# k-flouris/cmf

Hardware: AMD Instinct MI355X
Metric: log-density evals/sec (JtJ-cholesky path), MNIST D=784 d=64 bs=512 (higher is better)
Workload: dtype f32 (3x3 tangent convs as bf16x3 split MFMA, fp32 accumulate); 1 GPU; C3: MNIST-shaped (1,28,28) uint8-range + U[0,1) noise, non-square flow d=64, cholesky J^T J log-det + g_ij off-diagonal L1 + reconstruction, eval/no_grad; per_gpu_batch=512, global_batch=512, D=784, latent_dimension=64, parallelism=dp1

## Files before the change

### cmf_amd/_lib.py

```python
import ctypes as C
import os
import threading

_HERE = os.path.dirname(os.path.abspath(__file__))
LIB_PATH = os.path.join(_HERE, "libcmf_amd.so")

F_NONE, F_RELU, F_TANH, F_RAW, F_SELF_RELU, F_RELU_BITS = 0, 1, 2, 3, 4, 5
O_NONE, O_TANH, O_STANH = 0, 1, 2
GRAM_INVALID, GRAM_RING64, GRAM_DIRECT128, GRAM_WIDE, GRAM_RING_LIMIT = 0, 64, 128, 512, 0x7fffff00

_fp = C.c_void_p
_ll = C.c_longlong
_i = C.c_int
_f = C.c_float
_d = C.c_double


class ConvTangentArgs(C.Structure):
    _fields_ = [("x", _fp), ("x_np", _ll), ("x_ci", _ll), ("x_px", _ll),
                ("f", _fp), ("f_np", _ll), ("f_ci", _ll), ("f_px", _ll), ("fmode", _i),
                ("w", _fp),
                ("y", _fp), ("y_np", _ll), ("y_co", _ll), ("y_px", _ll),
                ("r", _fp), ("r_np", _ll), ("r_co", _ll), ("r_px", _ll),
                ("np", _i), ("cin", _i), ("cout", _i), ("H", _i), ("W", _i), ("nc", _i), ("taps", _i),
                ("bias", _fp), ("f_group", _i), ("x_sl", _ll), ("y_sl", _ll), ("r_sl", _ll),
                ("fo", _fp), ("fo_np", _ll), ("fo_co", _ll), ("fo_px", _ll), ("fomode", _i),
                ("mask_out", _fp), ("mask_np", _ll), ("amax_in", _fp), ("amax_out", _fp), ("live", _i),
                ("ymask", _fp), ("ymask_np", _ll),
                ("head_w", _fp), ("head_cout", _i), ("head_a", _fp), ("head_a_np", _ll), ("head_a_c", _ll), ("head_a_px", _ll),
                ("head_y", _fp), ("head_y_np", _ll), ("head_y_co", _ll), ("head_y_px", _ll),
                ("seed", _fp), ("seed_np", _ll), ("seed_col", _ll), ("seed_w", _fp),
                ("block_w1", _fp), ("block_m1", _fp), ("block_m1_np", _ll)]


class ConvPrimalArgs(C.Structure):
    _fields_ = [("x", _fp), ("x_b", _ll), ("x_c", _ll), ("x_px", _ll),
                ("f", _fp), ("f_c", _ll), ("f_px", _ll), ("imode", _i),
                ("w", _fp), ("bias", _fp), ("sw", _fp), ("sb", _fp),
                ("y", _fp), ("y_b", _ll), ("y_c", _ll), ("y_px", _ll),
                ("g", _fp),
                ("r", _fp), ("r_b", _ll), ("r_c", _ll), ("r_px", _ll),
                ("omode", _i),
                ("B", _i), ("cin", _i), ("cout", _i), ("H", _i), ("W", _i), ("taps", _i)]


class ProbeApplyArgs(C.Structure):
    _fields_ = [("r", _fp), ("r_np", _ll), ("r_px", _ll),
                ("t", _fp), ("t_np", _ll), ("t_c", _ll), ("t_px", _ll),
                ("cls", _fp),
                ("y", _fp), ("y_np", _ll), ("y_px", _ll),
                ("ymask", _fp), ("ymask_np", _ll),
                ("np", _i), ("cin", _i), ("H", _i), ("W", _i), ("nc", _i), ("ns", _i)]


MLP_MAX_LAYERS = 8
WGRAD_MAX_BATCH = 16


class MlpCouplerArgs(C.Structure):
    _fields_ = [("z", _fp), ("z_b", _ll), ("t", _fp), ("t_f", _ll), ("w", _fp),
                ("zi", _fp), ("si", _fp), ("ti", _fp), ("n_mod", _i),
                ("B", _i), ("cin", _i), ("chan_off", _i), ("chan_step", _i), ("n_layers", _i),
                ("width", _i * (MLP_MAX_LAYERS + 1)), ("w_off", _ll * MLP_MAX_LAYERS), ("decode", _i), ("lj", _fp), ("ncols", _i)]


SIGNATURES = {
    "cmf_version": (C.c_char_p, []),
    "cmf_pack_weight": (_i, [_fp, _fp, _i, _i, _i, _i, C.POINTER(_ll), _fp]),
    "cmf_pack_weights_batched": (_i, [_fp, _i, _fp]),
    "cmf_conv_tangent": (_i, [C.POINTER(ConvTangentArgs), _fp]),
    "cmf_pack_weight_bf16x3": (_i, [_fp, _fp, _i, _i, C.POINTER(_ll), _fp]),
    "cmf_pack_weight_bf16x3_t": (_i, [_fp, _fp, _i, _i, _i, C.POINTER(_ll), _fp]),
    "cmf_conv_tangent_bf16x3": (_i, [C.POINTER(ConvTangentArgs), _fp]),
    "cmf_probe_apply": (_i, [C.POINTER(ProbeApplyArgs), _fp]),
    "cmf_pack_seed_weight": (_i, [_fp, _fp, _fp]),
    "cmf_seed_panel": (_i, [_fp, _ll, _ll, _fp, _fp, _ll, _ll, _i, _i, _i, _i, _fp]),
    "cmf_pack_block_weight": (_i, [_fp, _fp, C.POINTER(_ll), _fp]),
    "cmf_pack_weight_f16x3": (_i, [_fp, _fp, _i, _i, _i, C.POINTER(_ll), _fp]),
    "cmf_conv_tangent_f16x3": (_i, [C.POINTER(ConvTangentArgs), _fp]),
    "cmf_conv_tangent_f16x3_item": (_i, [C.POINTER(ConvTangentArgs), _i, _fp]),
    "cmf_absmax": (_i, [_fp, _ll, _fp, _fp]),
    "cmf_conv_tangent_wgrad_ws": (_ll, [C.POINTER(ConvTangentArgs)]),
    "cmf_conv_tangent_wgrad": (_i, [C.POINTER(ConvTangentArgs), _fp, _fp, _fp, _ll, _fp]),
    "cmf_conv_tangent_wgrad_bf16x3": (_i, [C.POINTER(ConvTangentArgs), _fp, _fp, _fp, _ll, _fp]),
    "cmf_conv_tangent_wgrad_bf16x3_batched": (_i, [C.POINTER(ConvTangentArgs), _i, C.POINTER(_fp), C.POINTER(_fp), C.POINTER(_fp), _fp, _ll, _fp]),
    "cmf_primal_regroup": (_i, [_fp, _fp, _i, _ll, _i, _fp]),
    "cmf_conv_primal": (_i, [C.POINTER(ConvPrimalArgs), _fp]),
    "cmf_acl_primal": (_i, [_fp, _ll, _fp, _ll, _fp, _fp, _fp, _i, _i, _i, _fp, _fp]),
    "cmf_acl_tangent": (_i, [_fp, _ll, _ll, _fp, _ll, _ll, _i, _fp, _ll, _fp, _ll, _fp, _fp, _fp, _fp, _i, _i, _fp]),
    "cmf_acl_cotangent": (_i, [_fp, _ll, _ll, _fp, _ll, _ll, _i, _fp, _ll, _fp, _ll, _fp, _fp, _fp, _fp, _i, _i, _fp]),
    "cmf_acl_primal_backward": (_i, [_fp, _ll, _fp, _ll, _fp, _ll, _fp, _fp, _fp, _fp, _i, _i, _i, _fp, _fp]),
    "cmf_acl_cross_terms": (_i, [_fp, _ll, _ll, _fp, _ll, _ll, _fp, _ll, _ll, _i, _fp, _ll, _fp, _ll, _fp, _fp, _fp, _fp, _i, _i,
                            _fp, _fp, _fp, _fp]),
    "cmf_gather_primal": (_i, [_fp, _ll, _fp, _ll, _fp, _i, _i, _fp]),
    "cmf_gather_tangent": (_i, [_fp, _ll, _ll, _fp, _ll, _ll, _fp, _i, _i, _i, _fp]),
    "cmf_seed_tangent": (_i, [_fp, _ll, _ll, _fp, _i, _i, _fp, _i, _i, _i, _fp]),
    "cmf_gram_cholesky": (_i, [_fp, _ll, _ll, _i, _i, _i, _i, _fp, _fp, _fp, _fp, _fp, _fp, _fp]),
    "cmf_cholesky_retry": (_i, [_fp, _i, _i, _i, _f, _fp, _fp, _fp, _fp, _fp]),
    "cmf_gram_cholesky_family": (_i, [_i, _i, _ll]),
    "cmf_gram_condition": (_i, [_fp, _fp, _i, _i, _f, _fp, _fp, _fp, _fp, _fp]),
    "cmf_metric_stats_ws": (_ll, [_i, _i, _i, _i]),
    "cmf_metric_stats_accumulate": (_i, [_fp, _i, _i, _i, _fp, _fp, _ll, _fp, _fp]),
    "cmf_gram_spectrum": (_i, [_fp, _i, _i, _fp, _fp, _fp, _fp, _fp]),
    "cmf_gauss_newton_step": (_i, [_fp, _ll, _ll, _i, _i, _i, _i, _fp, _fp, _fp, _fp, _fp, _fp, _fp, _fp, _fp]),
    "cmf_cross_gram": (_i, [_fp, _ll, _ll, _i, _i, _i, _i, _i, _fp, _fp]),
    "cmf_curve_step_ws": (_ll, [_i, _i, _i]),
    "cmf_curve_step": (_i, [_fp, _ll, _ll, _i, _i, _i, _i, _i, _fp, _fp, _fp, _fp, _fp, _fp, _fp, _fp, _fp, _fp, _ll, _fp]),
    "cmf_stanh_backward": (_i, [_fp, _fp, _fp, _fp, _fp, _fp, _fp, _fp, _fp, _i, _i, _i, _fp]),
    "cmf_tanh_cross_terms": (_i, [_fp, _ll, _ll, _fp, _ll, _ll, _fp, _fp, _i, _i, _i, _fp]),
    "cmf_tanh_backward": (_i, [_fp, _fp, _fp, _ll, _fp, _fp]),
    "cmf_affine_prior_backward": (_i, [_fp, _ll, _fp, _ll, _fp, _i, _i, _fp, _fp, _fp, _fp]),
    "cmf_accumulate": (_i, [_fp, _fp, _ll, _fp]),
    "cmf_relu_bits": (_i, [_fp, _fp, _i, _i, _i, _fp]),
    "cmf_channel_sum": (_i, [_fp, _ll, _ll, _ll, _ll, _i, _i, _i, _i, _fp, _fp]),
    "cmf_channel_sum_batched": (_i, [C.POINTER(_fp), C.POINTER(_fp), _i, _ll, _ll, _ll, _ll, _i, _i, _i, _i, _fp]),
    "cmf_grad_sqnorm": (_i, [_fp, _ll, _fp, _fp, _fp]),
    "cmf_optimizer_step": (_i, [_i, _fp, _fp, _fp, _fp, _ll, _d, _d, _d, _d, _d, _i, _fp, _f, _fp]),
    "cmf_gram_backward_matrix": (_i, [_fp, _ll, _ll, _i, _i, _i, _i, _fp, _fp, _ll, _ll, _fp]),
    "cmf_gram_backward": (_i, [_fp, _ll, _ll, _i, _i, _i, _i, _fp, _fp, _fp, _fp, _fp, _ll, _ll, _fp]),
    "cmf_gram_backward_ws": (_i, [_fp, _ll, _ll, _i, _i, _i, _i, _fp, _fp, _fp, _fp, _fp, _ll, _ll, _fp, _fp]),
    "cmf_prehead": (_i, [_fp, _fp, _fp, _fp, _f, _f, _i, _i, _i, _fp]),
    "cmf_prehead_inverse": (_i, [_fp, _fp, _f, _f, _i, _ll, _fp]),
    "cmf_expand_columns": (_i, [_fp, _i, _fp, _i, _fp, _ll, _fp]),
    "cmf_gaussian_logprob": (_i, [_fp, _ll, _i, _i, _fp, _fp]),
    "cmf_affine_prior": (_i, [_fp, _ll, _fp, _fp, _i, _i, _i, _fp, _fp]),
    "cmf_recon_sqerr": (_i, [_fp, _fp, _i, _i, _fp, _fp]),
    "cmf_elbo_combine": (_i, [_fp, _fp, _fp, _fp, _fp, _f, _f, _f, _i, _fp, _fp]),
    "cmf_hutch_cg": (_i, [_fp, _fp, _i, _i, _i, _i, _i, _f, _fp, _fp, _fp, _fp, _fp]),
    "cmf_mlp_coupler": (_i, [C.POINTER(MlpCouplerArgs), _fp]),
    "cmf_pack_mlp_layer": (_i, [_fp, _fp, _i, _i, _i, _i, _i, _fp, C.POINTER(_ll), _fp]),
    "cmf_mlp_hidden_tiles": (_i, [_i]),
    "cmf_rq_spline": (_i, [_fp, _ll, _fp, _i, _i, _i, _f, _i, _i, _fp, _ll, _fp, _fp]),
    "cmf_rq_spline_backward": (_i, [_fp, _ll, _fp, _i, _i, _i, _f, _i, _fp, _ll, _fp, _fp, _ll, _fp, _fp]),
    "cmf_lu_backward": (_i, [_fp, _fp, _fp, _fp, _i, _f, _fp, _i, _fp, _fp, _fp, _fp, _fp]),
    "cmf_gaussian_backward": (_i, [_fp, _fp, _i, _i, _fp, _fp]),
    "cmf_lu_weights": (_i, [_fp, _fp, _fp, _i, _f, _fp, _fp, _fp]),
    "cmf_made_mask_weight": (_i, [_fp, _fp, _i, _i, _i, _i, _i, _fp]),
    "cmf_hutch_metric": (_i, [_fp, _i, _i, _i, _fp, _fp, _fp]),
    "cmf_hutch_cotangent": (_i, [_fp, _fp, _fp, _i, _i, _i, _fp, _fp, _fp, _fp, _fp]),
    "cmf_hutch_lowrank_cotangent": (_i, [_fp, _i, _i, _i, _fp, _fp, _i, _fp, _fp]),
}

_lib = None
_tls = threading.local()


class _Traced:

    def __init__(self, lib, sink):
        self._lib, self._sink = lib, sink

    def __getattr__(self, name):
        fn = getattr(self._lib, name)
        if not name.startswith("cmf_"):
            return fn
        import torch

        def call(*args):
            e0, e1 = torch.cuda.Event(enable_timing=True), torch.cuda.Event(enable_timing=True)
            e0.record()
            rc = fn(*args)
            e1.record()
            role = getattr(_tls, "role", None)
            self._sink.append((name + ":" + role if role else name, getattr(_tls, "phase", None), e0, e1))
            return rc
        return call


class trace:

    def __enter__(self):
        self.prev = getattr(_tls, "sink", None)
        _tls.sink = []
        return _tls.sink

    def __exit__(self, *exc):
        _tls.sink = self.prev
        return False


class phase:
    def __init__(self, label):
        self.label = label

    def __enter__(self):
        self.prev = getattr(_tls, "phase", None)
        if self.prev is None:
            _tls.phase = self.label

    def __exit__(self, *exc):
        _tls.phase = self.prev
        return False


def tracing():
    return getattr(_tls, "sink", None) is not None


class role:

    def __init__(self, label):
        self.label = label

    def __enter__(self):
        self.prev = getattr(_tls, "role", None)
        _tls.role = self.label

    def __exit__(self, *exc):
        _tls.role = self.prev
        return False


def load():
    global _lib
    sink = getattr(_tls, "sink", None)
    if _lib is not None:
        return _lib if sink is None else _Traced(_lib, sink)
    if not os.path.exists(LIB_PATH):
        raise RuntimeError(
            f"{LIB_PATH} is missing: the HIP kernels are the only implementation of this path "
            "(no CPU fallback). Build them with `python -m cmf_amd.build`.")
    lib = C.CDLL(LIB_PATH)
    for name, (res, args) in SIGNATURES.items():
        fn = getattr(lib, name)
        fn.restype, fn.argtypes = res, args
    _lib = lib
    return lib
# ... 7 lines not shown
```

### cmf_amd/csrc/probe_front.hip

```cpp
#include <stdint.h>

#include "common.h"

namespace {

constexpr int HID = 64, NT = 256, SLICE = HID * 16;
constexpr int MAXT = 50;
constexpr int MAXCLS = 32;
constexpr int PASS = 64;

__global__ __launch_bounds__(NT) void probe_apply_kernel(cmf_probe_apply_args a, int nitems) {
  __shared__ __attribute__((aligned(16))) float Rs[MAXCLS * HID];
  __shared__ __attribute__((aligned(16))) float Ts[MAXT * PASS];
  __shared__ int tcls[MAXT], toff[MAXT];
  __shared__ int nterm;

  const int per = (nitems + 7) >> 3;
  const int item = (int)(blockIdx.x & 7) * per + (int)(blockIdx.x >> 3);
  if (item >= nitems) return;
  const int H = a.H, W = a.W, HW = H * W;
  const int b = item / HW, p = item - b * HW;
  const int tid = threadIdx.x, lane = tid & 63, wv = tid >> 6;
  const int ncls = a.ns * 16;
  const f32x4 zero = {0.f, 0.f, 0.f, 0.f};

  unsigned long long live = ~0ull;
  if (a.ymask)
    live = *reinterpret_cast<const unsigned long long*>(reinterpret_cast<const unsigned char*>(a.ymask) + (long long)b * a.ymask_np +
                                                        (long long)p * (HID / 8));

  if (wv == 0) {
    int cls = -1, off = 0;
    if (lane < 25 * a.cin) {
      const int w = lane / a.cin, c = lane - w * a.cin;
      const int r = p / W + w / 5 - 2, col = p % W + w % 5 - 2;
      if (r >= 0 && r < H && col >= 0 && col < W) {
        const int q = r * W + col, k = a.cls[c * HW + q];
        if (k >= 0 && k < ncls) {
          cls = k;
          off = (int)(c * a.t_c + q * a.t_px);
        }
      }
    }
    const unsigned long long bal = __ballot(cls >= 0);
    if (cls >= 0) {
      const int pos = __popcll(bal & ((1ull << lane) - 1ull));
      tcls[pos] = cls;
      toff[pos] = off;
    }
    if (lane == 0) nterm = __popcll(bal);
  }

  {
    const int co = tid >> 2, k4 = (tid & 3) * 4;
    const float* rb = a.r + (long long)b * a.r_np + (long long)p * a.r_px + tid * 4;
    for (int s = 0; s < a.ns; ++s) {
      f32x4 v = zero;
      if ((live >> co) & 1) v = *reinterpret_cast<const f32x4*>(rb + s * SLICE);
#pragma unroll
      for (int m = 0; m < 4; ++m) Rs[(s * 16 + k4 + m) * HID + (co & 15) * 4 + (co >> 4)] = v[m];
    }
  }
  __syncthreads();

  const int n = nterm, nsl = a.nc >> 4, cg = lane >> 2, quad = lane & 3;
  const float* tb = a.t + (long long)b * a.t_np;
  for (int s0 = 0; s0 < nsl; s0 += PASS / 16) {
    const int w4 = (nsl - s0 < PASS / 16 ? nsl - s0 : PASS / 16) * 4;
    if (s0) __syncthreads();
    for (int i = tid; i < n * w4; i += NT) {
      const int j = i / w4, x = i - j * w4;
      *reinterpret_cast<f32x4*>(&Ts[j * PASS + 4 * x]) = *reinterpret_cast<const f32x4*>(tb + toff[j] + s0 * 16 + 4 * x);
    }
    __syncthreads();
    const int sl = s0 + wv;
    if (sl >= nsl) continue;
    f32x4 acc[4] = {zero, zero, zero, zero};
    for (int j = 0; j < n; ++j) {
      const f32x4 c4 = *reinterpret_cast<const f32x4*>(&Rs[tcls[j] * HID + cg * 4]);
      const f32x4 t4 = *reinterpret_cast<const f32x4*>(&Ts[j * PASS + wv * 16 + quad * 4]);
#pragma unroll
      for (int i = 0; i < 4; ++i)
#pragma unroll
        for (int k = 0; k < 4; ++k) acc[i][k] = fmaf(c4[i], t4[k], acc[i][k]);
    }
    float* yb = a.y + (long long)b * a.y_np + (long long)p * a.y_px + sl * SLICE + quad * 4;
#pragma unroll
    for (int i = 0; i < 4; ++i) {
      const int co = cg + 16 * i;
      if ((live >> co) & 1) *reinterpret_cast<f32x4*>(yb + co * 16) = acc[i];
    }
  }
}

bool fits_i32(long long v) { return v >= 0 && v <= 0x7fffffffLL; }

}

extern "C" int cmf_probe_apply(const cmf_probe_apply_args* ap, void* stream) {
  if (!ap) return CMF_EINVAL;
  const cmf_probe_apply_args& a = *ap;
  if (!a.r || !a.t || !a.cls || !a.y) return CMF_EINVAL;
  if (a.np <= 0 || a.H <= 0 || a.W <= 0 || a.nc <= 0 || a.nc % 16) return CMF_EINVAL;
  if (a.cin < 1 || 25 * a.cin > MAXT || a.ns < 1 || a.ns * 16 > MAXCLS) return CMF_EINVAL;
  if ((a.r_np | a.r_px | a.t_np | a.t_c | a.t_px | a.y_np | a.y_px) % 4) return CMF_EINVAL;
  if ((uintptr_t)a.r % 16 || (uintptr_t)a.t % 16 || (uintptr_t)a.y % 16) return CMF_EINVAL;
  if (a.r_np < 0 || a.t_np < 0 || a.y_np < 0 || a.t_c < 0) return CMF_EINVAL;
  if (a.r_px < (long long)a.ns * SLICE || a.y_px < (long long)HID * a.nc || a.t_px < a.nc) return CMF_EINVAL;
  const long long HW = (long long)a.H * a.W;
  if (a.ymask && ((uintptr_t)a.ymask % 8 || a.ymask_np % 8 || a.ymask_np < HW * (HID / 8))) return CMF_EINVAL;
  if (HW > (1 << 24) || !fits_i32(a.cin * a.t_c + HW * a.t_px + a.nc)) return CMF_ERANGE;
  const long long nitems = HW * a.np;
  if (nitems > 0x7ffffff0LL) return CMF_ERANGE;
  const int grid = 8 * (int)((nitems + 7) / 8);
  hipLaunchKernelGGL(probe_apply_kernel, dim3(grid), dim3(NT), 0, (hipStream_t)stream, a, (int)nitems);
  CMF_LAUNCH_CHECK();
  return 0;
}
```

### cmf_amd/engine.py

```python
import ctypes as C
import threading
from typing import NamedTuple

import numpy as np
import torch
import torch.nn as nn

from . import _lib
from ._lib import (F_NONE, F_RELU, F_TANH, F_RAW, F_SELF_RELU, F_RELU_BITS, O_NONE, O_TANH, O_STANH, ConvPrimalArgs,
                   ConvTangentArgs)


def _stream():
    return C.c_void_p(torch.cuda.current_stream().cuda_stream)


def _p(t):
    return None if t is None else C.c_void_p(t.data_ptr())


def require_gpu(t, what="input"):
    if not t.is_cuda:
        raise RuntimeError(f"cmf_amd: {what} is on {t.device}; the log-density path runs only through the HIP "
                           "kernels on an AMD GPU (there is no CPU fallback)")
# ... 1359 lines not shown
            a = a2
        y, g = new(cout), new(cout)
        conv_primal(a, 0, hid * HW, HW, 1, convf.weight, 1, convf.bias, y, cout * HW, HW, 1, B, hid, cout, H, W,
                    imode=F_RELU, omode=O_STANH, sw=net.weights.detach().reshape(-1), sb=net.bias.detach().reshape(-1), g=g)
        return y, g, acts
    lins = [m for m in net if isinstance(m, nn.Linear)]
    F_in = geo.C
    h, h_c, h_px, h_off, cin = z, view.chan_step, F_in, view.chan_off, view.cin
    acts = []
    for i, lin in enumerate(lins):
        last = i == len(lins) - 1
        out = torch.empty(B, lin.out_features, dtype=torch.float32, device=dev)
        conv_primal(h, h_off, 0, h_c, h_px, lin.weight, 1, lin.bias, out, 0, 1, lin.out_features, 1, cin, lin.out_features,
                    1, B, omode=O_NONE if last else O_TANH)
        if not last:
            acts.append(out)
        h, h_c, h_px, h_off, cin = out, 1, lin.out_features, 0, lin.out_features
    return h, None, acts


def net_primal_zero_input(net, view, B, device):
    rows = 16 if B % 16 == 0 else 1
    params = list(net.parameters())

    def build():
        z0 = torch.zeros(rows, *view.geom.shape, dtype=torch.float32, device=device)
        y, g, _ = net_primal(net, z0, view, need_acts=False)
        return y[:1].clone(), (None if g is None else g[:1].clone())

    return DERIVED.get((id(params[0]), "zero-input", rows, cfg().primal, str(device)), params, build)


class GroupedActs(list):
    f_group = 16


class BitMask:

    def __init__(self, B, HW, C, device):
        self.data = torch.empty(B, HW, C // 8, dtype=torch.uint8, device=device)
        self.np_bytes = HW * (C // 8)


class ActList(list):
    grouped = None


def train_acts_mode(net, view, B, T=None, nc=None):
    nc = T.nc if T is not None else nc
    if net.kind != "resnet" or B % 32 or cfg().primal == "bf16x3":
        return True
    conv0 = _resnet_parts(net)[0]
    hid, H, W = conv0.out_channels, view.geom.H, view.geom.W
    if hid % 64 or not _shape_ok_bf16x3(9, hid, W, True, H, hid):
        return True
    if nc is not None and (cfg().tangent != "bf16x3" or nc % 32):
        return True
    return "train"


def _resnet_primal_grouped(net, blocks, convf, a0, B, hid, cout, H, W, need_acts):
    HW, G, dev = H * W, B // 16, a0.device
    pn = (hid * HW * 16, HW * 16, 16)
    new = lambda: torch.empty(G * hid * HW * 16, dtype=torch.float32, device=dev)
    train = need_acts == "train"
    prec = cfg().primal
    if (prec == "f16x3" and hid % 64) or (prec in ("f16x3", "bf16x3") and hid > 64):
        prec = "f32"
    bits = (need_acts == "bits" or train) and prec != "bf16x3" and hid % 16 == 0
    a = primal_regroup(a0, True)
    acts, masks = [a], []
    rng = None
    if prec == "f16x3":
        rng = torch.zeros(2 * len(blocks) + 1, dtype=torch.float32, device=dev)
        absmax(a, rng[0:1])
    ax = lambda i: dict(amax_in=rng[i:i + 1], amax_out=rng[i + 1:i + 2]) if rng is not None else {}
    for k, blk in enumerate(blocks):
        c1, a2 = new(), new()
        m1, m2 = (BitMask(B, HW, hid, dev), BitMask(B, HW, hid, dev)) if bits else (None, None)
        mo = lambda m: dict(mask_out=m.data, mask_np=m.np_bytes) if m is not None else {}
        conv_tangent(a, 0, *pn, blk.conv1.weight, 9, c1, *pn, G, hid, hid, H, W, 16, fmode=F_SELF_RELU, bias=blk.conv1.bias,
                     precision=prec, **mo(m1), **ax(2 * k))
        conv_tangent(c1, 0, *pn, blk.conv2.weight, 9, a2, *pn, G, hid, hid, H, W, 16, fmode=F_SELF_RELU, bias=blk.conv2.bias,
                     res_t=a, precision=prec, **mo(m2), **ax(2 * k + 1))
        acts += [c1, a2]
        masks += [m1, m2]
        a = a2
    yg = torch.empty(G * cout * HW * 16, dtype=torch.float32, device=dev)
    gg = torch.empty_like(yg)
    conv_primal(a, 0, hid * HW * 16, HW * 16, 1, convf.weight, 1, convf.bias, yg, cout * HW * 16, HW * 16, 1, G, hid, cout,
                1, HW * 16, imode=F_RELU, omode=O_STANH, sw=net.weights.detach().reshape(-1), sb=net.bias.detach().reshape(-1),
                g=gg)
    y = primal_regroup(yg.view(G, -1), False).view(B, cout, H, W)
    g = primal_regroup(gg.view(G, -1), False).view(B, cout, H, W)
    if not need_acts:
        return y, g, None
    std_of = lambda t: primal_regroup(t.view(G, -1), False).view(B, hid, H, W)
    if train:
        out = ActList([a0] + masks[:-1] + [std_of(acts[-1])] if bits else [a0] + [std_of(t) for t in acts[1:]])
        out.grouped = acts
        return y, g, out
    if bits:
        return y, g, [a0] + masks[:-1] + [std_of(acts[-1])]
    return y, g, [a0] + [std_of(t) for t in acts[1:]]


def _view_rows(T, view):
    if T.layout == "panel":
        HW = view.geom.HW
        rows = T.data[: T.B * T.N * T.nc].view(T.B, T.N // HW, HW * T.nc)[:, view.chan_off::view.chan_step][:, :view.cin]
        out = Tangent(T.B, view.cin * HW, T.nc, "panel", T.data.device)
    else:
        rows = T.data[: T.B * T.N * T.nc].view(T.N, T.B * T.nc)[view.chan_off::view.chan_step][:view.cin]
        out = Tangent(T.B, view.cin, T.nc, "fmajor", T.data.device)
    out.data.view(rows.shape).copy_(rows)
    return out


CHECKERBOARD_TAIL = True
SKIP_DEAD_ROWS = True
FOLD_HEAD = True
FOLD_BLOCK = True
PROBE_FRONT = True
SEED_RESIDUAL = True
FOLD_BLOCK_SHAPES = ((28, 28, 2),)
PROBE_FRONT_SHAPES = {(28, 28, 1)}
PROBE_CLASSES = 13


def probe_plan(mask):
    mask = np.asarray(mask)
    if mask.ndim != 3:
        return None
    cin, H, W = mask.shape
    if not 1 <= cin <= 2:
        return None
    r, col = np.meshgrid(np.arange(H), np.arange(W), indexing="ij")
    cls = (np.mod(r - 5 * col, 2 * PROBE_CLASSES) >> 1)[None] + PROBE_CLASSES * np.arange(cin)[:, None, None]
    cls = np.where(mask != 0, cls, -1).astype(np.int8)
    for r0 in range(H):
        for c0 in range(W):
            win = cls[:, max(r0 - 2, 0):r0 + 3, max(c0 - 2, 0):c0 + 3].reshape(-1)
            win = win[win >= 0]
            if len(np.unique(win)) != len(win):
                return None
    ns = (PROBE_CLASSES * cin + 15) // 16
    flat = cls.reshape(-1)
    probes = np.zeros((cin * H * W, 16 * ns), dtype=np.float32)
    rows = np.flatnonzero(flat >= 0)
    probes[rows, flat[rows]] = 1.0
    return {"cls": flat, "ns": ns, "probes": probes}


def probe_apply(R, r_np, r_px, T, t_off, t_np, t_c, t_px, cls, y, y_np, y_px, np_, cin, H, W, nc, ns, ymask=None):
    a = _lib.ProbeApplyArgs()
    a.r = _p(R); a.r_np, a.r_px = int(r_np), int(r_px)
    a.t = C.c_void_p(T.data_ptr() + 4 * int(t_off)); a.t_np, a.t_c, a.t_px = int(t_np), int(t_c), int(t_px)
    a.cls = _p(cls)
    a.y = _p(y); a.y_np, a.y_px = int(y_np), int(y_px)
    if ymask is not None:
        a.ymask, a.ymask_np = _p(ymask.data), int(ymask.np_bytes)
    a.np, a.cin, a.H, a.W, a.nc, a.ns = int(np_), int(cin), int(H), int(W), int(nc), int(ns)
    launch = lambda: _lib.check(_lib.load().cmf_probe_apply(C.byref(a), _stream()), "cmf_probe_apply")
    TIMER = _timer()
    if TIMER is None:
        return launch()
    px = float(H) * W * np_
    TIMER.wrap(f"probe_apply_ci{cin}", 2.0 * PROBE_CLASSES * cin * 64 * nc * px, 4.0 * px * 64 * (nc + 16 * ns), launch)


def seed_plane(H, W):
    return ((H + 2) * (W + 2) + 1 + 3) // 4 * 4


def seed_panel(T, view, H, W):
    assert T.layout == "panel" and view.cin == 1
    B, nc, HW, col = T.B, T.nc, H * W, seed_plane(H, W)
    out = torch.empty(B * nc * col, dtype=torch.float32, device=T.data.device)
    v = C.c_void_p(T.data.data_ptr() + 4 * int(view.chan_off * HW * nc))
    launch = lambda: _lib.check(_lib.load().cmf_seed_panel(v, T.t_b, nc, _p(view.mask), _p(out), nc * col, col, B, H, W, nc, _stream()),
                                "cmf_seed_panel")
    TIMER = _timer()
    if TIMER is None:
        launch()
    else:
        TIMER.wrap("seed_panel", 0.0, 4.0 * B * nc * (col + HW), launch)
    return dict(panel=out, np=nc * col, col=col)


def seed_pack_host(w):
    w = np.asarray(w, dtype=np.float32).reshape(64, 9)
    out = np.zeros((4, 64, 4), dtype=np.float32)
    for kq in range(3):
        for j in range(3):
            out[:, 16 * kq:16 * kq + 16, j] = w[:, 3 * kq + j].reshape(4, 16)
    return out


def seed_panel_index(H, W):
    idx = np.full(seed_plane(H, W), -1, dtype=np.int64)
    r, c = np.meshgrid(np.arange(H), np.arange(W), indexing="ij")
    idx[((r + 1) * (W + 2) + c + 1).reshape(-1)] = (r * W + c).reshape(-1)
    return idx


def _seed_pack(conv0, dev):
    def build():
        w = conv0.weight.detach().contiguous()
        assert tuple(w.shape) == (64, 1, 3, 3) and w.dtype == torch.float32
        out = torch.empty(4096, dtype=torch.uint8, device=dev)
        _lib.check(_lib.load().cmf_pack_seed_weight(_p(w), _p(out), _stream()), "cmf_pack_seed_weight")
        return out

    return DERIVED.get((id(conv0.weight), "seed-residual", str(dev)), [conv0.weight], build)


def _block_pack(weight, dev):
    def build():
        w = weight.detach().contiguous()
        assert tuple(w.shape) == (64, 64, 3, 3) and w.dtype == torch.float32
        n = C.c_longlong(0)
        _lib.check(_lib.load().cmf_pack_block_weight(None, None, C.byref(n), None), "pack size")
        out = torch.empty(n.value, dtype=torch.uint8, device=dev)
        _lib.check(_lib.load().cmf_pack_block_weight(_p(w), _p(out), None, _stream()), "cmf_pack_block_weight")
        return out

    return DERIVED.get((id(weight), "fold-block", str(dev)), [weight], build)


def _probe_hidden(conv0, view, plan, H, W, hid, dev):
    HW, ncp = H * W, 16 * plan["ns"]

    def build():
        out = torch.empty(HW * hid * ncp, dtype=torch.float32, device=dev)
        conv_tangent(plan["probes"], 0, view.cin * HW * ncp, HW * ncp, ncp, conv0.weight, 9, out, hid * HW * ncp, 16, hid * ncp,
                     1, view.cin, hid, H, W, ncp, fmode=F_RAW, f=view.mask, f_np=0, f_ci=HW, f_px=1, y_sl=hid * 16)
        return out

    return DERIVED.get((id(conv0.weight), "probe-front", H, W, view.cin, str(dev)), [conv0.weight], build)


def probe_front(conv0, conv1, T, view, plan, factor, ymask, scratch, u, H, W):
    B, nc, HW, hid, dev = T.B, T.nc, H * W, conv1.out_channels, T.data.device
    assert hid == 64 and T.layout == "panel"
    ncp = 16 * plan["ns"]
    conv_tangent(_probe_hidden(conv0, view, plan, H, W, hid, dev), 0, 0, 16, hid * ncp, conv1.weight, 9, scratch,
                 hid * HW * ncp, 16, hid * ncp, B, hid, hid, H, W, ncp, x_sl=hid * 16, y_sl=hid * 16, ymask=ymask, **factor)
    probe_apply(scratch, hid * HW * ncp, hid * ncp, T.data, view.chan_off * HW * nc, T.t_b, view.chan_step * HW * nc, nc,
                plan["cls"], u, hid * HW * nc, hid * nc, B, view.cin, H, W, nc, plan["ns"], ymask=ymask)


class TangentPlan(NamedTuple):
    filt: bool
    front: str
    tail: str
    compact: bool


def resnet_tangent_plan(net, view, nc, layout, acts, training):
    conv0, blocks, convf = _resnet_parts(net)
    hid, cout, nb, H, W = conv0.out_channels, convf.out_channels, len(blocks), view.geom.H, view.geom.W
    if training or hid % 64 or not _use_bf16x3(9, hid, W, False, H, hid):
        return TangentPlan(False, "plain", "plain", False)
    filt = bool(SKIP_DEAD_ROWS)
    if nb == 0 or getattr(acts, "f_group", 1) != 1:
        return TangentPlan(filt, "plain", "plain", False)
    bits, live = (lambda i: isinstance(acts[i], BitMask)), view.live is not None
    head = FOLD_HEAD and live and hid == 64 and cout <= 8 and nc % 16 == 0 and bits(2 * nb - 1)
    block = head and FOLD_BLOCK and nb >= 2 and bits(2 * nb - 2) and (H, W, cout) in FOLD_BLOCK_SHAPES
    tail = "block" if block else "head" if head else "live" if CHECKERBOARD_TAIL and live else "plain"
    front, probe = "plain", view.probe
    if (PROBE_FRONT and probe is not None and hid == 64 and view.mask is not None and layout == "panel" and nc % 16 == 0
            and nc > 16 * probe["ns"] and (H, W, view.cin) in PROBE_FRONT_SHAPES):
        front = "seeded" if SEED_RESIDUAL and view.cin == 1 and nb >= 2 and bits(1) else "probe"
    return TangentPlan(filt, front, tail, bool(CHECKERBOARD_TAIL and live))


def net_tangent(net, T, view, acts, transpose_packs=False, save=None):
    if save is not None:
        save.append(_view_rows(T, view))
    return (_resnet_tangent if net.kind == "resnet" else _mlp_tangent)(net, T, view, acts, save)


def _resnet_tangent(net, T, view, acts, save):
    geo, B, nc, dev = view.geom, T.B, T.nc, T.data.device
    conv0, blocks, convf = _resnet_parts(net)
    hid, cout, H, W, HW, nb = conv0.out_channels, convf.out_channels, geo.H, geo.W, geo.HW, len(blocks)
    plan = resnet_tangent_plan(net, view, nc, T.layout, acts, save is not None)
    new = lambda c: Tangent(B, c * HW, nc, "panel", dev)
    hd, hsl = (hid * HW * nc, 16, hid * nc), hid * 16
    fg = getattr(acts, "f_group", 1)
    fs = dict(f_np=hid * HW * fg, f_ci=HW * fg, f_px=fg, f_group=fg)
    fk = lambda t: dict(fmode=F_RELU_BITS, f=t.data, f_np=t.np_bytes) if isinstance(t, BitMask) else dict(fmode=F_RELU, f=t, **fs)

    def folded(x, blk, factor, **kw):
        HWo = HW // 2 if plan.compact else HW
        yt = Tangent(B, cout * HWo, nc, "panel", dev, compact=plan.compact)
        conv_tangent(x.data, 0, *hd, blk.conv2.weight, 9, yt.data, cout * HWo * nc, HWo * nc, nc, B, hid, hid, H, W, nc, x_sl=hsl,
                     live=view.live["parity"] if plan.compact else 0, **kw, **factor)
        return yt

    u, h2, h = new(hid), new(hid), None
    if plan.front != "seeded":
        h = new(hid)
        conv_tangent(T.data, view.chan_off * HW * nc, T.t_b, view.chan_step * HW * nc, nc, conv0.weight, 9, h.data, *hd,
                     B, view.cin, hid, H, W, nc, fmode=F_RAW if view.mask is not None else F_NONE, f=view.mask, f_np=0,
                     f_ci=HW, f_px=1, y_sl=hsl)
    for k, blk in enumerate(blocks):
        a_in, c1, last = acts[2 * k], acts[2 * k + 1], k + 1 == nb
        ym = c1 if plan.filt and isinstance(c1, BitMask) else None
        if last and plan.tail == "block":
            return folded(h, blk, fk(a_in), head=dict(weight=convf.weight, act=acts[-1], conv1=dict(weight=blk.conv1.weight, mask=c1)))
        if k == 0 and plan.front != "plain":
            probe_front(conv0, blk.conv1, T, view, view.probe, fk(a_in), ym, h2.data, u.data, H, W)
        else:
            conv_tangent(h.data, 0, *hd, blk.conv1.weight, 9, u.data, *hd, B, hid, hid, H, W, nc, x_sl=hsl, y_sl=hsl, **fk(a_in),
# ... 284 lines not shown
```

### include/cmf_amd.h

```cpp
#ifndef CMF_AMD_H
#define CMF_AMD_H

#ifdef __cplusplus
extern "C" {
#endif

#define CMF_EINVAL (-1)
#define CMF_ERANGE (-2)

#define CMF_F_NONE 0
#define CMF_F_RELU 1
#define CMF_F_TANH 2
#define CMF_F_RAW  3
#define CMF_F_SELF_RELU 4
#define CMF_F_RELU_BITS 5

#define CMF_O_NONE  0
#define CMF_O_TANH  1
#define CMF_O_STANH 2

const char* cmf_version(void);

int cmf_pack_weight(const float* w, float* out, int cout, int cin, int taps, int transpose,
                    long long* out_floats, void* stream);

typedef struct {
  const float* w; void* out; long long total;
  int cout, cin, taps, transpose, kind, reserved;
} cmf_pack_desc;
int cmf_pack_weights_batched(const cmf_pack_desc* table, int n, void* stream);

typedef struct {
  const float* x; long long x_np, x_ci, x_px;
  const float* f; long long f_np, f_ci, f_px;
  int fmode;
  const float* w;
  float* y;       long long y_np, y_co, y_px;
  const float* r; long long r_np, r_co, r_px;
  int np, cin, cout, H, W, nc, taps;
  const float* bias;
  int f_group;
  long long x_sl, y_sl, r_sl;
  const float* fo; long long fo_np, fo_co, fo_px; int fomode;
  void* mask_out; long long mask_np;
  const float* amax_in; float* amax_out;
  int live;
  const void* ymask; long long ymask_np;
  const float* head_w; int head_cout;
  const float* head_a; long long head_a_np, head_a_c, head_a_px;
  float* head_y; long long head_y_np, head_y_co, head_y_px;
  const float* seed; long long seed_np, seed_col; const void* seed_w;
  const void* block_w1; const void* block_m1; long long block_m1_np;
} cmf_conv_tangent_args;
int cmf_conv_tangent(const cmf_conv_tangent_args* a, void* stream);

int cmf_pack_weight_bf16x3(const float* w, void* out, int cout, int cin, long long* out_bytes, void* stream);
int cmf_pack_weight_bf16x3_t(const float* w, void* out, int cout, int cin, int transpose, long long* out_bytes, void* stream);
int cmf_conv_tangent_bf16x3(const cmf_conv_tangent_args* a, void* stream);
int cmf_pack_seed_weight(const float* w, void* out, void* stream);
int cmf_pack_block_weight(const float* w, void* out, long long* out_bytes, void* stream);
int cmf_seed_panel(const float* v, long long v_np, long long v_px, const float* mask, float* out, long long out_np, long long out_col,
                   int np, int H, int W, int nc, void* stream);

typedef struct {
  const float* r; long long r_np, r_px;
  const float* t; long long t_np, t_c, t_px;
  const signed char* cls;
  float* y;       long long y_np, y_px;
  const void* ymask; long long ymask_np;
  int np, cin, H, W, nc, ns;
} cmf_probe_apply_args;
int cmf_probe_apply(const cmf_probe_apply_args* a, void* stream);

int cmf_pack_weight_f16x3(const float* w, void* out, int cout, int cin, int transpose, long long* out_bytes, void* stream);
int cmf_conv_tangent_f16x3(const cmf_conv_tangent_args* a, void* stream);
int cmf_conv_tangent_f16x3_item(const cmf_conv_tangent_args* a, int item_channels, void* stream);
int cmf_absmax(const float* x, long long n, float* out, void* stream);

long long cmf_conv_tangent_wgrad_ws(const cmf_conv_tangent_args* a);
int cmf_conv_tangent_wgrad(const cmf_conv_tangent_args* a, const float* gy, float* dw, float* ws, long long ws_bytes,
                           void* stream);
int cmf_conv_tangent_wgrad_bf16x3(const cmf_conv_tangent_args* a, const float* gy, float* dw, float* ws, long long ws_bytes,
                                  void* stream);
#define CMF_WGRAD_MAX_BATCH 16
int cmf_conv_tangent_wgrad_bf16x3_batched(const cmf_conv_tangent_args* a, int nprob, const float* const* x, const float* const* gy,
                                          float* const* dw, float* ws, long long ws_bytes, void* stream);

typedef struct {
  const float* x; long long x_b, x_c, x_px;
  const float* f; long long f_c, f_px;
  int imode;
  const float* w; const float* bias;
  const float* sw; const float* sb;
  float* y;       long long y_b, y_c, y_px;
  float* g;
  const float* r; long long r_b, r_c, r_px;
  int omode;
  int B, cin, cout, H, W, taps;
} cmf_conv_primal_args;
int cmf_conv_primal(const cmf_conv_primal_args* a, void* stream);

int cmf_primal_regroup(const float* in, float* out, int B, long long N, int to_grouped, void* stream);

int cmf_acl_primal(float* z, long long z_b, const float* y, long long y_b, const int* zi, const int* si,
                   const int* ti, int n_mod, int B, int decode, float* lj, void* stream);
int cmf_acl_cotangent(float* c, long long c_b, long long c_r, float* yc, long long yc_b, long long yc_r, int nc,
                      const float* z, long long z_b, const float* y, long long y_b, const float* g, const int* zi,
                      const int* si, const int* ti, int n_mod, int B, void* stream);
int cmf_acl_primal_backward(float* dx, long long dx_b, const float* z, long long z_b, const float* y, long long y_b, float* dy,
                            const int* zi, const int* si, const int* ti, int n_mod, int B, int decode, const float* dlj,
                            void* stream);
int cmf_acl_cross_terms(const float* c, long long c_b, long long c_r, const float* v, long long v_b, long long v_r,
                        const float* yt, long long yt_b, long long yt_r, int nc, const float* z, long long z_b,
                        const float* y, long long y_b, const float* g, const int* zi, const int* si, const int* ti,
                        int n_mod, int B, float* dz, float* dy, float* dg, void* stream);
int cmf_acl_tangent(float* t, long long t_b, long long t_r, const float* yt, long long yt_b, long long yt_r,
                    int nc, const float* z, long long z_b, const float* y, long long y_b, const float* g,
                    const int* zi, const int* si, const int* ti, int n_mod, int B, void* stream);

int cmf_gather_primal(const float* in, long long in_b, float* out, long long out_b, const int* idx,
                      int n_out, int B, void* stream);
int cmf_gather_tangent(const float* in, long long in_b, long long in_r, float* out, long long out_b,
                       long long out_r, const int* idx, int n_out, int nc, int B, void* stream);
int cmf_expand_columns(const float* in, int nc_in, float* out, int nc_out, const int* colmap, long long rows, void* stream);
int cmf_seed_tangent(float* t, long long t_b, long long t_r, const int* col_of, int n_rows, int nc,
                     const float* eps, int d, int S, int B, void* stream);

int cmf_gram_cholesky(const float* t, long long t_b, long long t_r, int n_rows, int nc, int d, int B,
                      float* jtj, float* logdet, float* l1_off, float* l1_diag, int* info, int* fail,
                      void* stream);
int cmf_cholesky_retry(float* jtj, int d, int B, int attempt, float eps0, float* logdet, float* l1_diag,
                       int* info, int* fail, void* stream);
#define CMF_GRAM_INVALID   0
#define CMF_GRAM_STAGED1   1
#define CMF_GRAM_STAGED8   8
#define CMF_GRAM_RING64    64
#define CMF_GRAM_DIRECT128 128
#define CMF_GRAM_WIDE      512
#define CMF_GRAM_RING_LIMIT 0x7fffff00LL
int cmf_gram_cholesky_family(int n_rows, int nc, long long t_r);
int cmf_gram_condition(const float* jtj, const int* info, int d, int B, float threshold, float* cond, int* flagged_idx,
                       int* flagged_count, float* ws, void* stream);
long long cmf_metric_stats_ws(int d, int B, int chunk, int with_sample_macs);
int cmf_metric_stats_accumulate(const float* jtj, int d, int B, int chunk, double* state, double* ws, long long ws_doubles,
                                float* sample_macs, void* stream);
#define CMF_SPECTRUM_MAX_SWEEPS 64
int cmf_gram_spectrum(const float* jtj, int d, int B, double* eigenvalues, double* vectors, int* sweeps, int* info, void* stream);
int cmf_gauss_newton_step(const float* t, long long t_b, long long t_r, int n_rows, int nc, int d, int B,
                          const float* jtj, const float* x, const float* xhat, const double* damping,
                          double* grad, double* delta, double* stats, int* info, void* stream);
int cmf_cross_gram(const float* t, long long t_b, long long t_r, int n_rows, int nc, int d, int points, int curves, float* cross,
                   void* stream);
long long cmf_curve_step_ws(int d, int points, int curves);
int cmf_curve_step(const float* t, long long t_b, long long t_r, int n_rows, int nc, int d, int points, int curves,
                   const float* jtj, const float* cross, const float* xhat, const double* damping, double* grad, double* delta,
                   double* stats, double* seg2, int* info, double* ws, long long ws_doubles, void* stream);
int cmf_gram_backward(const float* t, long long t_b, long long t_r, int n_rows, int nc, int d, int B,
                      const float* jtj, const float* g_logdet, const float* g_l1off, const float* g_l1diag,
                      float* dt, long long dt_b, long long dt_r, void* stream);
int cmf_gram_backward_ws(const float* t, long long t_b, long long t_r, int n_rows, int nc, int d, int B,
                         const float* jtj, const float* g_logdet, const float* g_l1off, const float* g_l1diag,
                         float* dt, long long dt_b, long long dt_r, float* ws, void* stream);
int cmf_gram_backward_matrix(const float* t, long long t_b, long long t_r, int n_rows, int nc, int d, int B,
                             const float* m, float* dt, long long dt_b, long long dt_r, void* stream);

int cmf_prehead(const float* x, const float* u, float* y, float* lj, float a, float c, int logit, int n,
                int B, void* stream);
int cmf_prehead_inverse(const float* y, float* x, float a, float c, int logit, long long n_total, void* stream);
int cmf_gaussian_logprob(const float* z, long long z_b, int n, int B, float* lp, void* stream);
int cmf_affine_prior(float* z, long long z_b, const float* log_scale, const float* shift, int n, int B,
                     int decode, float* lj, void* stream);
int cmf_recon_sqerr(const float* xh, const float* x, int n, int B, float* rec, void* stream);
int cmf_elbo_combine(const float* low, const float* logdet, const float* rec, const float* l1, const float* pre,
                     float wl, float lam, float wm, int B, float* elbo, void* stream);
int cmf_hutch_cg(const float* jtj, const float* eps, int d, int S, int B, int max_iter, int min_iter, float tol,
                 float* u, float* w, float* val, int* iters, void* stream);
int cmf_hutch_metric(const float* w, int d, int S, int B, float* l1_off, float* l1_diag, void* stream);
int cmf_hutch_cotangent(const float* u, const float* eps, const float* w, int d, int S, int B, const float* g_val,
                        const float* g_off, const float* g_diag, float* M, void* stream);
int cmf_hutch_lowrank_cotangent(const float* w, int d, int S, int B, const float* g_val, const float* g_diag, int n,
                                float* cmat, void* stream);

#define CMF_MLP_MAX_LAYERS 8
typedef struct {
  float* z; long long z_b;
  float* t; long long t_f;
  const float* w;
  const int* zi; const int* si; const int* ti; int n_mod;
  int B, cin, chan_off, chan_step;
  int n_layers;
  int width[CMF_MLP_MAX_LAYERS + 1];
  long long w_off[CMF_MLP_MAX_LAYERS];
  int decode;
  float* lj;
  int ncols;
} cmf_mlp_coupler_args;
int cmf_mlp_coupler(const cmf_mlp_coupler_args* a, void* stream);
int cmf_pack_mlp_layer(const float* w, const float* bias, int out_features, int in_features, int first, int out_tiles,
                       int in_groups, float* out, long long* out_floats, void* stream);
int cmf_mlp_hidden_tiles(int max_hidden_width);

int cmf_rq_spline(const float* x, long long x_b, const float* params, int D, int bins, int hidden, float tail_bound,
                  int inverse, int B, float* out, long long out_b, float* lj, void* stream);
int cmf_rq_spline_backward(const float* x, long long x_b, const float* params, int D, int bins, int hidden, float tail_bound,
                           int B, const float* dz, long long dz_b, const float* dlj, float* dx, long long dx_b,
                           float* dparams, void* stream);
int cmf_lu_backward(const float* dW, const float* lower, const float* upper, const float* unconstrained_diag, int n, float eps,
                    const float* dlj, int B, float* scratch1, float* g_lower, float* g_upper, float* g_udiag, void* stream);
int cmf_gaussian_backward(const float* u, const float* dlow, int n, int B, float* du, void* stream);
int cmf_lu_weights(const float* lower, const float* upper, const float* unconstrained_diag, int n, float eps, float* W,
                   float* logdet, void* stream);
int cmf_made_mask_weight(const float* w, float* out, int n_out, int n_in, int kind, int features, int multiplier,
                         void* stream);

int cmf_stanh_backward(const float* dy, const float* dg, const float* y, const float* g, const float* sw,
                       const float* sb, float* du, float* dsw, float* dsb, int B, int C, int HW, void* stream);
int cmf_tanh_cross_terms(float* c, long long c_b, long long c_r, const float* x, long long x_b, long long x_r,
                         const float* h, float* dh, int F, int B, int nc, void* stream);
int cmf_tanh_backward(const float* dh, const float* a, const float* extra, long long n, float* out, void* stream);
int cmf_affine_prior_backward(float* dz, long long dz_b, const float* x, long long x_b, const float* log_scale, int n, int B,
                              const float* dlj, float* g_ls, float* g_sh, void* stream);
int cmf_accumulate(float* dst, const float* src, long long n, void* stream);
int cmf_relu_bits(const float* act, void* out, int B, int C, int HW, void* stream);
int cmf_channel_sum(const float* t, long long t_np, long long t_c, long long t_px, long long t_sl, int np, int C,
                    int npx, int nc, float* out, void* stream);
// ... 16 lines not shown
```

Measured before the change: 1557 evals/s.

## Process probe-apply in 14-pixel row strips with shared T window and double-buffered R

Replaces the per-pixel probe_apply kernel with a strip kernel in which each workgroup handles up to 14 consecutive pixels of a row. The 5x(strip+4) tangent window and class map are staged once in LDS and reused across the overlapping 5x5 neighbourhoods, where the old kernel reloaded them for every pixel. Per-pixel R coefficients are double-buffered with software prefetch, and the inner loop iterates only over live taps found by a wave ballot. The old kernel is kept as a reference entry point. The cost is more dynamic LDS, lower occupancy and a __syncthreads per pixel.

```diff
diff --git a/cmf_amd/_lib.py b/cmf_amd/_lib.py
--- a/cmf_amd/_lib.py
+++ b/cmf_amd/_lib.py
@@ -73,6 +73,7 @@
     "cmf_pack_weight_bf16x3_t": (_i, [_fp, _fp, _i, _i, _i, C.POINTER(_ll), _fp]),
     "cmf_conv_tangent_bf16x3": (_i, [C.POINTER(ConvTangentArgs), _fp]),
     "cmf_probe_apply": (_i, [C.POINTER(ProbeApplyArgs), _fp]),
+    "cmf_probe_apply_ref": (_i, [C.POINTER(ProbeApplyArgs), _fp]),
     "cmf_pack_seed_weight": (_i, [_fp, _fp, _fp]),
     "cmf_seed_panel": (_i, [_fp, _ll, _ll, _fp, _fp, _ll, _ll, _i, _i, _i, _i, _fp]),
     "cmf_pack_block_weight": (_i, [_fp, _fp, C.POINTER(_ll), _fp]),
diff --git a/cmf_amd/csrc/probe_front.hip b/cmf_amd/csrc/probe_front.hip
--- a/cmf_amd/csrc/probe_front.hip
+++ b/cmf_amd/csrc/probe_front.hip
@@ -93,11 +93,158 @@
   }
 }
 
+constexpr int STRIP = 14;
+constexpr int SW = STRIP + 4, WPOS = 5 * SW;
+constexpr int TU = 3;
+
+int strip_lds(int cin, int ns) { return (cin * WPOS * PASS + 2 * ns * 16 * HID) * 4 + (STRIP + 2) * 8 + cin * WPOS * 4; }
+
+template <int NS>
+__global__ __launch_bounds__(NT, NS == 1 ? 5 : 4) void probe_apply_strip_kernel(cmf_probe_apply_args a, int nitems, int nstrip) {
+  extern __shared__ __attribute__((aligned(16))) float lds[];
+  constexpr int ncls = NS * 16;
+  const int cin = a.cin;
+  float* Ts = lds;
+  float* Rs = Ts + cin * WPOS * PASS;
+  uint2* lives = reinterpret_cast<uint2*>(Rs + 2 * ncls * HID);
+  int* clsS = reinterpret_cast<int*>(lives + STRIP + 2);
+
+  const int per = (nitems + 7) >> 3;
+  const int item = (int)(blockIdx.x & 7) * per + (int)(blockIdx.x >> 3);
+  if (item >= nitems) return;
+  const int H = a.H, W = a.W, HW = H * W;
+  const int b = item / (H * nstrip), rs = item - b * (H * nstrip);
+  const int row = rs / nstrip, x0 = (rs - row * nstrip) * STRIP;
+  const int npx = W - x0 < STRIP ? W - x0 : STRIP, p0 = row * W + x0;
+  const int tid = threadIdx.x, lane = tid & 63, wv = tid >> 6;
+  const int cg = lane >> 2, quad = lane & 3, co_b = tid >> 2, k4 = (tid & 3) * 4;
+  const int nsl = a.nc >> 4;
+  const f32x4 zero = {0.f, 0.f, 0.f, 0.f};
+  const unsigned char* ym = reinterpret_cast<const unsigned char*>(a.ymask) + (long long)b * a.ymask_np + (long long)p0 * (HID / 8);
+  const float* rb = a.r + (long long)b * a.r_np + (long long)p0 * a.r_px + tid * 4;
+  const float* tb = a.t + (long long)b * a.t_np;
+
+  auto live_word = [&](int px) -> uint2 {
+    if (px >= npx) return make_uint2(0u, 0u);
+    return a.ymask ? *reinterpret_cast<const uint2*>(ym + px * (HID / 8)) : make_uint2(~0u, ~0u);
+  };
+  auto uniform = [](uint2 lv) -> uint2 {
+    return make_uint2(__builtin_amdgcn_readfirstlane(lv.x), __builtin_amdgcn_readfirstlane(lv.y));
+  };
+  auto live_bit = [](uint2 lv, int co) -> bool { return ((co & 32 ? lv.y : lv.x) >> (co & 31)) & 1; };
+  auto load_r = [&](int px, uint2 lv, f32x4 (&v)[NS]) {
+    if (live_bit(lv, co_b)) {
+#pragma unroll
+      for (int s = 0; s < NS; ++s) v[s] = *reinterpret_cast<const f32x4*>(rb + (long long)px * a.r_px + s * SLICE);
+    }
+  };
+  auto write_r = [&](int buf, uint2 lv, const f32x4 (&v)[NS]) {
+    float* dst = Rs + buf * ncls * HID + k4 * HID + (co_b & 15) * 4 + (co_b >> 4);
+    const bool on = live_bit(lv, co_b);
+#pragma unroll
+    for (int s = 0; s < NS; ++s)
+#pragma unroll
+      for (int m = 0; m < 4; ++m) dst[(s * 16 + m) * HID] = on ? v[s][m] : 0.f;
+  };
+
+  int wofs = -1;
+  if (lane < 25 * cin) {
+    const int w = lane / cin, c = lane - w * cin;
+    wofs = (c * 5 + w / 5) * SW + w % 5;
+  }
+
+  for (int s0 = 0; s0 < nsl; s0 += PASS / 16) {
+    const int w4 = (nsl - s0 < PASS / 16 ? nsl - s0 : PASS / 16) * 4;
+    const bool active = s0 + wv < nsl;
+    f32x4 r0[NS], rv[NS];
+    const uint2 lv0 = live_word(0), lv1 = live_word(1);
+    load_r(0, lv0, r0);
+    load_r(1, lv1, rv);
+
+    if (tid < STRIP + 2) lives[tid] = live_word(tid);
+    for (int i = tid; i < cin * WPOS; i += NT) {
+      const int c = i / WPOS, wr = (i - c * WPOS) / SW, wc = i - c * WPOS - wr * SW;
+      const int r = row + wr - 2, col = x0 + wc - 2;
+      int k = -1;
+      if (r >= 0 && r < H && col >= 0 && col < W && wc < npx + 4) k = a.cls[c * HW + r * W + col];
+      clsS[i] = k >= 0 && k < ncls ? k : -1;
+    }
+    for (int i0 = 0; i0 < cin * WPOS * 16; i0 += NT * TU) {
+      int src[TU];
+      f32x4 v[TU];
+#pragma unroll
+      for (int u = 0; u < TU; ++u) {
+        const int i = i0 + u * NT + tid, pos = i >> 4, x = i & 15;
+        const int c = pos / WPOS, wr = (pos - c * WPOS) / SW, wc = pos - c * WPOS - wr * SW;
+        const int r = row + wr - 2, col = x0 + wc - 2;
+        src[u] = -1;
+        if (pos < cin * WPOS && x < w4 && r >= 0 && r < H && col >= 0 && col < W && wc < npx + 4) {
+          const int q = r * W + col, k = a.cls[c * HW + q];
+          if (k >= 0 && k < ncls) src[u] = (int)(c * a.t_c + q * a.t_px) + s0 * 16 + 4 * x;
+        }
+      }
+#pragma unroll
+      for (int u = 0; u < TU; ++u)
+        if (src[u] >= 0) v[u] = *reinterpret_cast<const f32x4*>(tb + src[u]);
+#pragma unroll
+      for (int u = 0; u < TU; ++u)
+        if (src[u] >= 0) *reinterpret_cast<f32x4*>(&Ts[(i0 + u * NT + tid) * 4]) = v[u];
+    }
+    write_r(0, lv0, r0);
+    __syncthreads();
+
+    int kn = wofs >= 0 ? clsS[wofs] : -1;
+    float* yb = a.y + (long long)b * a.y_np + (long long)p0 * a.y_px + (s0 + wv) * SLICE + quad * 4;
+    for (int i = 0; i < npx; ++i) {
+      const int kc = kn;
+      if (i + 1 < npx) kn = wofs >= 0 ? clsS[wofs + i + 1] : -1;
+      const uint2 live = uniform(lives[i]), live1 = uniform(lives[i + 1]), live2 = uniform(lives[i + 2]);
+      f32x4 acc[4] = {zero, zero, zero, zero};
+      if (active) {
+        const float* rc = Rs + (i & 1) * ncls * HID + cg * 4;
+        const float* tc = Ts + i * PASS + wv * 16 + quad * 4;
+        unsigned long long bal = __ballot(kc >= 0);
+        auto fetch = [&](f32x4& c4, f32x4& t4) {
+          const int l = __builtin_ctzll(bal);
+          bal &= bal - 1;
+          c4 = *reinterpret_cast<const f32x4*>(rc + __builtin_amdgcn_readlane(kc, l) * HID);
+          t4 = *reinterpret_cast<const f32x4*>(tc + __builtin_amdgcn_readlane(wofs, l) * PASS);
+        };
+        auto fma16 = [&](const f32x4& c4, const f32x4& t4) {
+#pragma unroll
+          for (int j = 0; j < 4; ++j)
+#pragma unroll
+            for (int k = 0; k < 4; ++k) acc[j][k] = fmaf(c4[j], t4[k], acc[j][k]);
+        };
+        if (bal) {
+          f32x4 c4, t4, c4n, t4n;
+          fetch(c4, t4);
+          while (bal) {
+            fetch(c4n, t4n);
+            fma16(c4, t4);
+            c4 = c4n;
+            t4 = t4n;
+          }
+          fma16(c4, t4);
+        }
+      }
+      write_r((i + 1) & 1, live1, rv);
+      load_r(i + 2, live2, rv);
+      if (active) {
+#pragma unroll
+        for (int j = 0; j < 4; ++j) {
+          const int co = cg + 16 * j;
+          if (live_bit(live, co)) *reinterpret_cast<f32x4*>(yb + (long long)i * a.y_px + co * 16) = acc[j];
+        }
+      }
+      __syncthreads();
+    }
+  }
+}
+
 bool fits_i32(long long v) { return v >= 0 && v <= 0x7fffffffLL; }
 
-}
-
-extern "C" int cmf_probe_apply(const cmf_probe_apply_args* ap, void* stream) {
+int probe_apply_check(const cmf_probe_apply_args* ap) {
   if (!ap) return CMF_EINVAL;
   const cmf_probe_apply_args& a = *ap;
   if (!a.r || !a.t || !a.cls || !a.y) return CMF_EINVAL;
@@ -110,10 +257,31 @@
   const long long HW = (long long)a.H * a.W;
   if (a.ymask && ((uintptr_t)a.ymask % 8 || a.ymask_np % 8 || a.ymask_np < HW * (HID / 8))) return CMF_EINVAL;
   if (HW > (1 << 24) || !fits_i32(a.cin * a.t_c + HW * a.t_px + a.nc)) return CMF_ERANGE;
-  const long long nitems = HW * a.np;
-  if (nitems > 0x7ffffff0LL) return CMF_ERANGE;
+  if (HW * a.np > 0x7ffffff0LL) return CMF_ERANGE;
+  return 0;
+}
+
+}
+
+extern "C" int cmf_probe_apply_ref(const cmf_probe_apply_args* ap, void* stream) {
+  if (const int rc = probe_apply_check(ap)) return rc;
+  const cmf_probe_apply_args& a = *ap;
+  const long long nitems = (long long)a.H * a.W * a.np;
   const int grid = 8 * (int)((nitems + 7) / 8);
   hipLaunchKernelGGL(probe_apply_kernel, dim3(grid), dim3(NT), 0, (hipStream_t)stream, a, (int)nitems);
   CMF_LAUNCH_CHECK();
   return 0;
 }
+
+extern "C" int cmf_probe_apply(const cmf_probe_apply_args* ap, void* stream) {
+  if (const int rc = probe_apply_check(ap)) return rc;
+  const cmf_probe_apply_args& a = *ap;
+  static_assert((2 * WPOS * PASS + 2 * MAXCLS * HID) * 4 + (STRIP + 2) * 8 + 2 * WPOS * 4 <= 65536, "strip item beyond a plain launch's LDS");
+  const int nstrip = (a.W + STRIP - 1) / STRIP;
+  const long long nitems = (long long)a.H * nstrip * a.np;
+  const int grid = 8 * (int)((nitems + 7) / 8);
+  hipLaunchKernelGGL(a.ns == 1 ? probe_apply_strip_kernel<1> : probe_apply_strip_kernel<2>, dim3(grid), dim3(NT), strip_lds(a.cin, a.ns),
+                     (hipStream_t)stream, a, (int)nitems, nstrip);
+  CMF_LAUNCH_CHECK();
+  return 0;
+}
diff --git a/cmf_amd/engine.py b/cmf_amd/engine.py
--- a/cmf_amd/engine.py
+++ b/cmf_amd/engine.py
@@ -1535,7 +1535,7 @@
     return {"cls": flat, "ns": ns, "probes": probes}
 
 
-def probe_apply(R, r_np, r_px, T, t_off, t_np, t_c, t_px, cls, y, y_np, y_px, np_, cin, H, W, nc, ns, ymask=None):
+def probe_apply(R, r_np, r_px, T, t_off, t_np, t_c, t_px, cls, y, y_np, y_px, np_, cin, H, W, nc, ns, ymask=None, ref=False):
     a = _lib.ProbeApplyArgs()
     a.r = _p(R); a.r_np, a.r_px = int(r_np), int(r_px)
     a.t = C.c_void_p(T.data_ptr() + 4 * int(t_off)); a.t_np, a.t_c, a.t_px = int(t_np), int(t_c), int(t_px)
@@ -1544,7 +1544,8 @@
     if ymask is not None:
         a.ymask, a.ymask_np = _p(ymask.data), int(ymask.np_bytes)
     a.np, a.cin, a.H, a.W, a.nc, a.ns = int(np_), int(cin), int(H), int(W), int(nc), int(ns)
-    launch = lambda: _lib.check(_lib.load().cmf_probe_apply(C.byref(a), _stream()), "cmf_probe_apply")
+    symbol = "cmf_probe_apply_ref" if ref else "cmf_probe_apply"
+    launch = lambda: _lib.check(getattr(_lib.load(), symbol)(C.byref(a), _stream()), symbol)
     TIMER = _timer()
     if TIMER is None:
         return launch()
diff --git a/include/cmf_amd.h b/include/cmf_amd.h
--- a/include/cmf_amd.h
+++ b/include/cmf_amd.h
@@ -71,6 +71,7 @@
   int np, cin, H, W, nc, ns;
 } cmf_probe_apply_args;
 int cmf_probe_apply(const cmf_probe_apply_args* a, void* stream);
+int cmf_probe_apply_ref(const cmf_probe_apply_args* a, void* stream);
 
 int cmf_pack_weight_f16x3(const float* w, void* out, int cout, int cin, int transpose, long long* out_bytes, void* stream);
 int cmf_conv_tangent_f16x3(const cmf_conv_tangent_args* a, void* stream);
```

Result: no change. 1562 evals/s (median of 6 runs) (+0.3%).
